# joeyee/Onet

Measured on AMD Instinct MI355X. Metric: training images/sec (twin 256x256 pass), higher is better.
Workload: dtype f32

## Files before the change

### onet_amd/csrc/conv_split.hip

```cpp
#include <algorithm>
#include <cstdlib>
#include "common.hpp"

using namespace onet;

typedef float f32x16 __attribute__((ext_vector_type(16)));
typedef __bf16 bf16x8 __attribute__((ext_vector_type(8)));
typedef __bf16 bf16x2 __attribute__((ext_vector_type(2)));
typedef unsigned int u32x4s __attribute__((ext_vector_type(4)));
typedef float f32x4s __attribute__((ext_vector_type(4)));

namespace {

constexpr unsigned OOB_S = 0x80000000u;

__device__ __forceinline__ __amdgpu_buffer_rsrc_t s_rsrc(const void* base, int64_t bytes) {
    const int n = bytes > 0x7fffffffll ? 0x7fffffff : (int)bytes;
    return __builtin_amdgcn_make_buffer_rsrc(const_cast<void*>(base), 0, n, 0x00020000);
}
__device__ __forceinline__ void split2(float a, float b, unsigned& hi, unsigned& mid) {
    const bf16x2 h = {(__bf16)a, (__bf16)b};
    const bf16x2 m = {(__bf16)(a - (float)h[0]), (__bf16)(b - (float)h[1])};
    hi = __builtin_bit_cast(unsigned, h);
    mid = __builtin_bit_cast(unsigned, m);
// ... 693 lines not shown
            }
#pragma unroll
            for (int idx = 0; idx < 9; ++idx) {
                const int kx = idx / 3, ky = idx % 3;
                if (idx < 8) {
                    const int nt = ((idx + 1) % 3) * 3 + (idx + 1) / 3;
#pragma unroll
                    for (int m = 0; m < 2; ++m) {
                        Aq[(idx + 1) & 1][m][0] = ab[nt * 2 * CO_T + m * 32];
                        Aq[(idx + 1) & 1][m][1] = ab[nt * 2 * CO_T + m * 32 + W_PART];
                    }
                }
                if (kx < 2) {
#pragma unroll
                    for (int j = 0; j < NB; ++j)
                        if (j % 3 == ky) {
                            Bq[(kx + 1) & 1][j][0] = bb[j * IN_COLS + kx + 1];
                            Bq[(kx + 1) & 1][j][1] = bb[j * IN_COLS + kx + 1 + IN_PART];
                        }
                }
                if (idx == 0) advance();
                {
                    constexpr int NPIECE = NII + NWI, PER = (NPIECE + C::LAST_TAP) / (C::LAST_TAP + 1);
#pragma unroll
                    for (int q = 0; q < PER; ++q) {
                        const int pc = idx * PER + q;
                        if (idx <= C::LAST_TAP && pc < NPIECE) {
                            if (pc & 1) { if (pc / 2 < NWI) dma_w(buf ^ 1, pc / 2); else dma_in(buf ^ 1, pc - NWI); }
                            else { if (pc / 2 < NII) dma_in(buf ^ 1, pc / 2); else dma_w(buf ^ 1, pc - NII); }
                        }
                    }
                }
                __builtin_amdgcn_sched_barrier(0);
#pragma unroll
                for (int m = 0; m < 2; ++m)
#pragma unroll
                    for (int n = 0; n < NT; ++n) {
                        if constexpr (PM == 2) {
                            const bf16x8 a0 = __builtin_bit_cast(bf16x8, Aq[idx & 1][m][0]), a1 = __builtin_bit_cast(bf16x8, Aq[idx & 1][m][1]);
                            const bf16x8 b0 = __builtin_bit_cast(bf16x8, Bq[kx & 1][n + ky][0]), b1 = __builtin_bit_cast(bf16x8, Bq[kx & 1][n + ky][1]);
                            acc[m][n] = __builtin_amdgcn_mfma_f32_32x32x16_bf16(a0, b0, acc[m][n], 0, 0, 0);
                            acc[m][n] = __builtin_amdgcn_mfma_f32_32x32x16_bf16(a1, b1, acc[m][n], 0, 0, 0);
                        } else if constexpr (F16) {
                            const f16x8 ah = __builtin_bit_cast(f16x8, Aq[idx & 1][m][0]), am = __builtin_bit_cast(f16x8, Aq[idx & 1][m][1]);
                            const f16x8 bh = __builtin_bit_cast(f16x8, Bq[kx & 1][n + ky][0]), bm = __builtin_bit_cast(f16x8, Bq[kx & 1][n + ky][1]);
                            acc[m][n] = __builtin_amdgcn_mfma_f32_32x32x16_f16(am, bh, acc[m][n], 0, 0, 0);
                            acc[m][n] = __builtin_amdgcn_mfma_f32_32x32x16_f16(ah, bm, acc[m][n], 0, 0, 0);
                            acc[m][n] = __builtin_amdgcn_mfma_f32_32x32x16_f16(ah, bh, acc[m][n], 0, 0, 0);
                        } else {
                            const bf16x8 ah = __builtin_bit_cast(bf16x8, Aq[idx & 1][m][0]), am = __builtin_bit_cast(bf16x8, Aq[idx & 1][m][1]);
                            const bf16x8 bh = __builtin_bit_cast(bf16x8, Bq[kx & 1][n + ky][0]), bm = __builtin_bit_cast(bf16x8, Bq[kx & 1][n + ky][1]);
                            acc[m][n] = __builtin_amdgcn_mfma_f32_32x32x16_bf16(am, bh, acc[m][n], 0, 0, 0);
                            acc[m][n] = __builtin_amdgcn_mfma_f32_32x32x16_bf16(ah, bm, acc[m][n], 0, 0, 0);
                            acc[m][n] = __builtin_amdgcn_mfma_f32_32x32x16_bf16(ah, bh, acc[m][n], 0, 0, 0);
                        }
                    }
                __builtin_amdgcn_sched_barrier(0);
            }
            asm volatile("s_waitcnt vmcnt(0)" ::: "memory");
            __syncthreads();
            buf ^= 1;
        }

#pragma unroll
        for (int m = 0; m < 2; ++m)
#pragma unroll
            for (int n = 0; n < NT; ++n)
#pragma unroll
                for (int r = 0; r < 16; ++r) acc[m][n][r] *= acc_scale;
        const auto [co0, tx, ty, b, y0, x0] = sp_tile(tile, a.coTiles, a.tilesX, a.tilesY);
        if constexpr (ST) {
            float* sc = reinterpret_cast<float*>(lds + 2 * BUF);
            constexpr float npw = (float)(NT * 32), inv_npw = 1.f / npw;
#pragma unroll
            for (int m = 0; m < 2; ++m)
#pragma unroll
                for (int r = 0; r < 16; ++r) {
                    const int piv = __builtin_bit_cast(int, acc[m][0][r]);
                    const float p0 = __builtin_bit_cast(float, __builtin_amdgcn_readlane(piv, 0));
                    const float p1 = __builtin_bit_cast(float, __builtin_amdgcn_readlane(piv, 32));
                    const float pv = kh ? p1 : p0;
                    float s1 = 0.f, s2 = 0.f;
#pragma unroll
                    for (int n = 0; n < NT; ++n) {
                        const float d = acc[m][n][r] - pv;
                        s1 += d;
                        s2 = fmaf(d, d, s2);
                    }
                    s1 = sp_half_sum(s1);
                    s2 = sp_half_sum(s2);
                    if (l31 == 31) {
                        const int cl = m * 32 + (r & 3) + 8 * (r >> 2) + 4 * kh;
                        sc[(wn * 64 + cl) * 2] = fmaf(s1, inv_npw, pv);
                        sc[(wn * 64 + cl) * 2 + 1] = fmaxf(fmaf(-s1 * inv_npw, s1, s2), 0.f);
                    }
                }
            __syncthreads();
            if (tid < 64 && co0 + tid < a.Cout) {
                float mw[8], qw[8];
#pragma unroll
                for (int w = 0; w < 8; ++w) {
                    mw[w] = sc[(w * 64 + tid) * 2];
                    qw[w] = sc[(w * 64 + tid) * 2 + 1];
                }
                const float mean = 0.125f * (((mw[0] + mw[1]) + (mw[2] + mw[3])) + ((mw[4] + mw[5]) + (mw[6] + mw[7])));
                float m2 = ((qw[0] + qw[1]) + (qw[2] + qw[3])) + ((qw[4] + qw[5]) + (qw[6] + qw[7]));
#pragma unroll
                for (int w = 0; w < 8; ++w) m2 = fmaf(npw * (mw[w] - mean), mw[w] - mean, m2);
                const int64_t nblk = (int64_t)a.B * a.tilesY * a.tilesX;
                const int64_t blk = ((int64_t)b * a.tilesY + ty) * a.tilesX + tx;
                float* sp = a.stats + ((int64_t)(co0 + tid) * nblk + blk) * 3;
                sp[0] = 8.f * npw;
                sp[1] = mean;
                sp[2] = m2;
            }
            __syncthreads();
        }
        float* zb = a.z + (int64_t)(W16 ? 2 * b + (l31 >> 4) : b) * a.z_bs;
        const int xo = W16 ? (l31 & 15) : x0 + l31;
        if constexpr (ACT) {
            const float* cf = act_cf + cf_par * 192;
            float vmax = 0.f;
#pragma unroll
            for (int m = 0; m < 2; ++m)
#pragma unroll
                for (int g = 0; g < 4; ++g) {
                    const int cl = m * 32 + 8 * g + 4 * kh;
                    const f32x4s mean = *reinterpret_cast<const f32x4s*>(cf + cl);
                    const f32x4s sc = *reinterpret_cast<const f32x4s*>(cf + 64 + cl);
                    const f32x4s sh = *reinterpret_cast<const f32x4s*>(cf + 128 + cl);
#pragma unroll
                    for (int n = 0; n < NT; ++n)
#pragma unroll
                        for (int j = 0; j < 4; ++j) {
                            const float v = fmaxf(fmaf(acc[m][n][4 * g + j] - mean[j], sc[j], sh[j]), 0.f);
                            acc[m][n][4 * g + j] = v;
                            vmax = fmaxf(vmax, v);
                        }
                }
            if (a.act_amax) {
#pragma unroll
                for (int o = 32; o > 0; o >>= 1) vmax = fmaxf(vmax, __shfl_xor(vmax, o, 64));
                if (lane == 0 && vmax == vmax)
                    atomicMax(a.act_amax + ((tile * NWV + wn) & (AMAX_SLOTS - 1)) * AMAX_STRIDE, __builtin_bit_cast(unsigned, vmax));
            }
            if (a.act_a) {
                float* ab = a.act_a + (int64_t)b * a.act_a_bs;
#pragma unroll
                for (int m = 0; m < 2; ++m)
#pragma unroll
                    for (int n = 0; n < NT; ++n) {
                        const int yo = y0 + wn * NT + n;
                        if (yo < a.H && xo < a.W) {
#pragma unroll
                            for (int r = 0; r < 16; ++r) {
                                const int co = co0 + m * 32 + (r & 3) + 8 * (r >> 2) + 4 * kh;
                                if (co < a.Cout) ab[(int64_t)co * HW + (int64_t)yo * a.W + xo] = acc[m][n][r];
                            }
                        }
                    }
            }
        }
        if constexpr (PM == 1 && !ST && !W16) {
            if (ACT || (a.zP && co0 >= a.zP_ch0)) {
                const float zs = zP_scale;
                u32x4s* zp = reinterpret_cast<u32x4s*>(reinterpret_cast<unsigned*>(a.zP) + (int64_t)b * a.zP_bs);
#pragma unroll
                for (int m = 0; m < 2; ++m)
#pragma unroll
                    for (int n = 0; n < NT; ++n) {
                        const int yo = y0 + wn * NT + n;
#pragma unroll
                        for (int e = 0; e < 2; ++e) {
                            float v[8];
#pragma unroll
                            for (int j = 0; j < 4; ++j) {
                                const float f0 = acc[m][n][8 * e + j], f1 = acc[m][n][8 * e + 4 + j];
                                const unsigned d0 = __builtin_bit_cast(unsigned, f0);
                                const unsigned d1 = __builtin_bit_cast(unsigned, f1);
                                const auto sw = __builtin_amdgcn_permlane32_swap(d0, d1, false, false);
                                const unsigned lo = sw[0], hi4 = sw[1];
                                v[j] = __builtin_bit_cast(float, lo);
                                v[4 + j] = __builtin_bit_cast(float, hi4);
                            }
                            u32x4s hi, mid;
#pragma unroll
                            for (int k = 0; k < 4; ++k) {
                                unsigned hh, mm;
                                split2h_s(v[2 * k], v[2 * k + 1], zs, hh, mm);
                                hi[k] = hh;
                                mid[k] = mm;
                            }
                            if (yo < a.H && xo < a.W) {
                                const int c8 = ((co0 - a.zP_ch0 + m * 32) >> 3) + 2 * e + kh;
                                u32x4s* d = zp + ((int64_t)(c8 * a.H + yo) * 2) * a.W + xo;
                                d[0] = hi;
                                d[a.W] = mid;
                            }
                        }
                    }
                continue;
            }
        }
#pragma unroll
        for (int m = 0; m < 2; ++m)
#pragma unroll
            for (int n = 0; n < NT; ++n) {
                const int yo = y0 + wn * NT + n;
                if (yo < a.H && xo < a.W) {
#pragma unroll
                    for (int r = 0; r < 16; ++r) {
                        const int co = co0 + m * 32 + (r & 3) + 8 * (r >> 2) + 4 * kh;
                        if (co < a.Cout) zb[(int64_t)co * HW + (int64_t)yo * a.W + xo] = acc[m][n][r];
                    }
                }
            }
    }
}


template <bool ST, int PM, bool W16, bool RD = false>
__global__ __launch_bounds__(512, 2) void conv3x3_pre16_kernel(SpPreArgs a) {
    constexpr bool F16 = PM == 1;
    using C = SpPreCfg<W16>;
    static_assert(C::NW == 8 && C::NT == 2, "conv3x3_pre16_kernel: 8 waves of 2 rows");
    constexpr int NT = 2, IN_COLS = C::IN_COLS, NWI = C::NWI, CO_T = C::CO_T, NPIXP = C::NPIXP;
    constexpr int BUF = C::BUF_SLOTS, IN_PART = C::IN_PART;
    constexpr int NII = (2 * IN_PART + 511) / 512;
    constexpr int CH_OFF = W16 ? 18 : 16;
    constexpr int NSTEP = PM == 2 ? 9 : 14;
    extern __shared__ __attribute__((aligned(16))) unsigned char smem_s[];
    u32x4s* lds = reinterpret_cast<u32x4s*>(smem_s);

    int t_first, t_end, t_stride;
    sp_tile_range(a.tilesX * a.tilesY * a.B * a.coTiles, t_first, t_end, t_stride);
    if (t_first >= t_end) return;

    const int tid = threadIdx.x, lane = tid & 63, wn = __builtin_amdgcn_readfirstlane(tid >> 6);
    const int r16 = lane & 15, lq = lane >> 4, hq = lq & 1, gq = lq >> 1;
    const int HW = a.H * a.W;
    const int nchunks = PM == 2 ? a.Cin >> 5 : a.Cin >> 4;

    const i32x4s wr = sp_rsrc4(a.wq, (int64_t)a.Cin * (PM == 2 ? 1 : 2) * 9 * a.Cout * 2);
    float xs_inv = 1.f, xs_inv2 = 1.f;
    (void)amax_scale(amax_read(a.x_slots), a.x_always != 0, xs_inv);
    (void)amax_scale(amax_read(a.x_slots2), a.x_always != 0, xs_inv2);
    const int split_chunk = a.split_ch ? (PM == 2 ? a.split_ch >> 5 : a.split_ch >> 4) : 0;
    const float grp_ratio = split_chunk ? xs_inv / xs_inv2 : 1.f;
    const float acc_scale = (split_chunk ? xs_inv2 : xs_inv) * (F16 ? reinterpret_cast<const float*>(a.wq + (int64_t)a.Cin * 2 * 9 * a.Cout)[1] : 1.f);
    const unsigned in_step = (unsigned)(16 * HW * 4), w_step = (unsigned)(2 * 9 * 2 * a.Cout * 16);
    const unsigned lds0 = (unsigned)(uintptr_t)(__attribute__((address_space(3))) unsigned char*)smem_s;

    unsigned in_off[NII], w_off[NWI];
    i32x4s xr;
    int st_tile = t_first, st_chunk = 0;
    unsigned cin_bytes = 0, cw_bytes = 0;
    auto setup_stage = [&]() __attribute__((always_inline)) {
        const bool live = st_tile < t_end;
        const auto [co0, tx, ty, b, y0, x0] = sp_tile(live ? st_tile : t_first, a.coTiles, a.tilesX, a.tilesY);
        xr = sp_rsrc4(reinterpret_cast<const unsigned*>(a.xs) + (int64_t)(W16 ? 2 * b : b) * a.xs_bs,
                      (W16 ? a.xs_bs * 4 : 0) + (int64_t)a.Cin * HW * (PM == 2 ? 2 : 4));
#pragma unroll
        for (int k = 0; k < NII; ++k) {
            const int i = (wn + 8 * k) * 64 + lane;
            const int ph = i / NPIXP, pix = i % NPIXP;
            const int r = pix / IN_COLS, c = pix % IN_COLS;
            const int img = W16 ? c / 18 : 0;
            const int yy = y0 - 1 + r, xx = W16 ? c % 18 - 1 : x0 - 1 + c;
            const bool ok = live && i < 2 * IN_PART && pix < C::NPIX && yy >= 0 && yy < a.H && xx >= 0 && xx < a.W;
            const unsigned io = W16 ? (unsigned)(img * a.xs_bs * 4) : 0u;
            in_off[k] = !ok ? OOB_S : PM == 2 ? io + (unsigned)(((ph * a.H + yy) * a.W + xx) * 16)
                                              : io + (unsigned)(((((ph & 1) * a.H + yy) * 2 + (ph >> 1)) * a.W + xx) * 16);
        }
#pragma unroll
        for (int k = 0; k < NWI; ++k) {
            const int i = tid + 512 * k;
            const int co = i & (CO_T - 1), pth = i >> 6;
            const bool ok = live && (i < C::W_SLOTS) && (co0 + co < a.Cout);
            w_off[k] = ok ? (unsigned)((pth * a.Cout + co0 + co) * 16) : OOB_S;
        }
    };
    auto advance = [&]() __attribute__((always_inline)) {
        ++st_chunk;
        cin_bytes += in_step;
        cw_bytes += w_step;
        if (st_chunk == nchunks) {
            st_chunk = 0;
            cin_bytes = cw_bytes = 0;
            st_tile += t_stride;
            setup_stage();
        }
    };
    auto dma_in = [&](int buf, int k) __attribute__((always_inline)) {
        if ((wn + 8 * k) * 64 < 2 * IN_PART)
            sp_dma16(xr, lds0 + (unsigned)((buf * BUF + C::W_SLOTS + (wn + 8 * k) * 64) * 16), in_off[k], cin_bytes);
    };
    auto dma_w = [&](int buf, int k) __attribute__((always_inline)) {
        if (k < NWI - 1 || wn < (C::W_SLOTS - 512 * (NWI - 1)) / 64)
            sp_dma16(wr, lds0 + (unsigned)((buf * BUF + (wn + 8 * k) * 64) * 16), w_off[k], cw_bytes);
    };

    const int xrow0 = (wn * NT) * IN_COLS + r16;
    const u32x4s* const xa_p = lds + C::W_SLOTS + (PM == 2 ? lq : hq) * NPIXP + xrow0;
    const u32x4s* const xh_p = lds + C::W_SLOTS + (2 + hq) * NPIXP + xrow0 + gq;
    const u32x4s* const xv_p = lds + C::W_SLOTS + (2 + hq) * NPIXP + xrow0 + gq * IN_COLS + 2;
    const u32x4s* const xs_p = lds + C::W_SLOTS + (2 + hq) * NPIXP + xrow0 + 2;
    const u32x4s* const wa_p = lds + (gq * 9 * 2 + hq) * CO_T + r16;
    const u32x4s* const wh_p = lds + (gq * 2 + hq) * CO_T + r16;
    const u32x4s* const wv_p = lds + ((3 * gq + 2) * 2 + hq) * CO_T + r16;
    const u32x4s* const ws_p = gq == 0 ? lds + (8 * 2 + hq) * CO_T + r16 : lds + C::W_SLOTS + C::NPIX;
    const int ws_ct = gq == 0 ? 16 : 0;

    setup_stage();
#pragma unroll
    for (int k = 0; k < NII; ++k) dma_in(0, k);
#pragma unroll
    for (int k = 0; k < NWI; ++k) dma_w(0, k);
    asm volatile("s_waitcnt vmcnt(0)" ::: "memory");
    __syncthreads();
    int buf = 0;
    for (int tile = t_first; tile < t_end; tile += t_stride) {
        f32x4s acc[4][NT][2];
#pragma unroll
        for (int ct = 0; ct < 4; ++ct)
#pragma unroll
            for (int n = 0; n < NT; ++n)
#pragma unroll
                for (int ch = 0; ch < 2; ++ch) acc[ct][n][ch] = f32x4s{0.f, 0.f, 0.f, 0.f};

        for (int c = 0; c < nchunks; ++c) {
            if (split_chunk && c == split_chunk && grp_ratio != 1.f) {
#pragma unroll
                for (int ct = 0; ct < 4; ++ct)
#pragma unroll
                    for (int n = 0; n < NT; ++n)
#pragma unroll
                        for (int ch = 0; ch < 2; ++ch) acc[ct][n][ch] *= grp_ratio;
            }
            const int bo = buf * BUF;
            u32x4s Xp[2][NT + 2][2], Wf[2][4];
            auto load_x = [&](int ph, int f) __attribute__((always_inline)) {
                const int j = f >> 1, ch = f & 1, p = ph & 1;
                if (ph < 3) Xp[p][j][ch] = xa_p[bo + j * IN_COLS + ch * CH_OFF + ph];
                else if (ph == 3) Xp[p][j][ch] = xh_p[bo + j * IN_COLS + ch * CH_OFF];
                else if (j < NT) Xp[p][j][ch] = xv_p[bo + j * IN_COLS + ch * CH_OFF];
                else Xp[p][j][ch] = xs_p[bo + j * IN_COLS + ch * CH_OFF];
            };
            auto load_w = [&](int s) __attribute__((always_inline)) {
#pragma unroll
                for (int ct = 0; ct < 4; ++ct) {
                    if (s < 9) Wf[s & 1][ct] = wa_p[bo + ((s % 3) * 3 + s / 3) * 2 * CO_T + ct * 16];
                    else if (s < 12) Wf[s & 1][ct] = wh_p[bo + (s - 9) * 6 * CO_T + ct * 16];
                    else if (s == 12) Wf[s & 1][ct] = wv_p[bo + ct * 16];
                    else Wf[s & 1][ct] = ws_p[bo + ct * ws_ct];
                }
            };
#pragma unroll
            for (int f = 0; f < 2 * (NT + 2); ++f) load_x(0, f);
            load_w(0);
#pragma unroll
            for (int s = 0; s < NSTEP; ++s) {
                const int ph = s < 9 ? s / 3 : (s < 12 ? 3 : 4);
                const int ro = s < 9 ? s % 3 : (s < 12 ? s - 9 : (s == 12 ? 0 : NT));
                if (s + 1 < NSTEP) load_w(s + 1);
                if (s < 12 && ph + 1 < (PM == 2 ? 3 : 5)) {
#pragma unroll
                    for (int f = 0; f < 2 * (NT + 2); ++f)
                        if (f % 3 == s % 3) load_x(ph + 1, f);
                }
                if (s == 0) advance();
                {
                    constexpr int NPIECE = NII + NWI, PER = (NPIECE + C::LAST_TAP) / (C::LAST_TAP + 1);
#pragma unroll
                    for (int q = 0; q < PER; ++q) {
                        const int pc = s * PER + q;
                        if (s <= C::LAST_TAP && pc < NPIECE) {
                            if (pc & 1) { if (pc / 2 < NWI) dma_w(buf ^ 1, pc / 2); else dma_in(buf ^ 1, pc - NWI); }
                            else { if (pc / 2 < NII) dma_in(buf ^ 1, pc / 2); else dma_w(buf ^ 1, pc - NII); }
                        }
                    }
                }
                __builtin_amdgcn_sched_barrier(0);
#pragma unroll
                for (int ct = 0; ct < 4; ++ct)
#pragma unroll
                    for (int n = 0; n < NT; ++n)
#pragma unroll
                        for (int ch = 0; ch < 2; ++ch) {
                            if constexpr (F16)
                                acc[ct][n][ch] = __builtin_amdgcn_mfma_f32_16x16x32_f16(__builtin_bit_cast(f16x8, Xp[ph & 1][ro + n][ch]),
                                                                                        __builtin_bit_cast(f16x8, Wf[s & 1][ct]), acc[ct][n][ch], 0, 0, 0);
                            else
                                acc[ct][n][ch] = __builtin_amdgcn_mfma_f32_16x16x32_bf16(__builtin_bit_cast(bf16x8, Xp[ph & 1][ro + n][ch]),
                                                                                         __builtin_bit_cast(bf16x8, Wf[s & 1][ct]), acc[ct][n][ch], 0, 0, 0);
                        }
                __builtin_amdgcn_sched_barrier(0);
            }
            asm volatile("s_waitcnt vmcnt(0)" ::: "memory");
            __syncthreads();
            buf ^= 1;
        }

#pragma unroll
        for (int ct = 0; ct < 4; ++ct)
#pragma unroll
            for (int n = 0; n < NT; ++n)
#pragma unroll
                for (int ch = 0; ch < 2; ++ch) acc[ct][n][ch] *= acc_scale;
        const auto [co0, tx, ty, b, y0, x0] = sp_tile(tile, a.coTiles, a.tilesX, a.tilesY);
        if constexpr (ST) {
            float* sc = reinterpret_cast<float*>(lds + (buf ^ 1) * BUF);
            constexpr float npw = (float)(NT * 32);
#pragma unroll
            for (int ct = 0; ct < 4; ++ct) {
                const float pv = acc[ct][0][0][0];
                float s1 = 0.f, s2 = 0.f;
#pragma unroll
                for (int n = 0; n < NT; ++n)
#pragma unroll
                    for (int ch = 0; ch < 2; ++ch)
#pragma unroll
                        for (int r = 0; r < 4; ++r) {
                            const float d = acc[ct][n][ch][r] - pv;
                            s1 += d;
                            s2 = fmaf(d, d, s2);
                        }
                float mean = fmaf(s1, 1.f / 16.f, pv), m2 = fmaxf(fmaf(-s1 * (1.f / 16.f), s1, s2), 0.f), cnt = 16.f;
#pragma unroll
                for (int o = 16; o <= 32; o <<= 1) {
                    const float mo = __shfl_xor(mean, o, 64), qo = __shfl_xor(m2, o, 64);
                    const float dlt = mo - mean;
                    m2 = (m2 + qo) + (0.5f * cnt) * dlt * dlt;
                    mean = 0.5f * (mean + mo);
                    cnt *= 2.f;
                }
                if (lq == 0) {
                    sc[(wn * 64 + ct * 16 + r16) * 2] = mean;
                    sc[(wn * 64 + ct * 16 + r16) * 2 + 1] = m2;
                }
            }
            __syncthreads();
            if (tid < 64 && co0 + tid < a.Cout) {
                float mw[8], qw[8];
#pragma unroll
                for (int w = 0; w < 8; ++w) {
                    mw[w] = sc[(w * 64 + tid) * 2];
                    qw[w] = sc[(w * 64 + tid) * 2 + 1];
                }
                const float mean = 0.125f * (((mw[0] + mw[1]) + (mw[2] + mw[3])) + ((mw[4] + mw[5]) + (mw[6] + mw[7])));
                float m2 = ((qw[0] + qw[1]) + (qw[2] + qw[3])) + ((qw[4] + qw[5]) + (qw[6] + qw[7]));
#pragma unroll
                for (int w = 0; w < 8; ++w) m2 = fmaf(npw * (mw[w] - mean), mw[w] - mean, m2);
                const int64_t nblk = (int64_t)a.B * a.tilesY * a.tilesX;
                const int64_t blk = ((int64_t)b * a.tilesY + ty) * a.tilesX + tx;
                float* sp = a.stats + ((int64_t)(co0 + tid) * nblk + blk) * 3;
                sp[0] = 8.f * npw;
                sp[1] = mean;
                sp[2] = m2;
            }
            __syncthreads();
        }
        f32x4s zr[4][NT][2];
        const float* rd_sv = nullptr;
        if constexpr (RD) {
            const int img0 = W16 ? 2 * b : b;
            rd_sv = a.rd_save + (int64_t)(a.rd_gimg ? img0 / a.rd_gimg : 0) * 4 * a.Cout;
#pragma unroll
            for (int ct = 0; ct < 4; ++ct)
#pragma unroll
                for (int n = 0; n < NT; ++n)
#pragma unroll
                    for (int ch = 0; ch < 2; ++ch) {
                        const int co = co0 + ct * 16 + r16, yo = y0 + wn * NT + n, xo = (W16 ? 0 : x0 + 16 * ch) + 4 * lq;
                        f32x4s zz = {0.f, 0.f, 0.f, 0.f};
                        if (co < a.Cout && yo < a.H && xo < a.W) {
                            const int64_t zo = (int64_t)(W16 ? img0 + ch : img0) * a.rd_z_bs + (int64_t)co * HW + (int64_t)yo * a.W + xo;
                            if (a.rd_z16) {
                                const uint2 u = *reinterpret_cast<const uint2*>(reinterpret_cast<const __bf16*>(a.rd_z) + zo);
                                zz = f32x4s{__builtin_bit_cast(float, u.x << 16), __builtin_bit_cast(float, u.x & 0xffff0000u),
                                            __builtin_bit_cast(float, u.y << 16), __builtin_bit_cast(float, u.y & 0xffff0000u)};
                            } else {
                                zz = *reinterpret_cast<const f32x4s*>(a.rd_z + zo);
                            }
                        }
                        zr[ct][n][ch] = zz;
                    }
            __builtin_amdgcn_sched_barrier(0);
        }
        {
            const int half = r16 >> 3, c8 = r16 & 7;
            float* zb = a.z + (int64_t)(W16 ? 2 * b + half : b) * a.z_bs;
            const int xo = (W16 ? 0 : x0 + 16 * half) + 4 * lq;
#pragma unroll
            for (int n = 0; n < NT; ++n) {
                const int yo = y0 + wn * NT + n;
#pragma unroll
                for (int ct = 0; ct < 4; ++ct) {
                    const i32x4s va = __builtin_bit_cast(i32x4s, acc[ct][n][0]), vb = __builtin_bit_cast(i32x4s, acc[ct][n][1]);
                    const i32x4s e1 = {__builtin_amdgcn_update_dpp(va.x, vb.x, 0x128, 0xf, 0xc, false), __builtin_amdgcn_update_dpp(va.y, vb.y, 0x128, 0xf, 0xc, false),
                                       __builtin_amdgcn_update_dpp(va.z, vb.z, 0x128, 0xf, 0xc, false), __builtin_amdgcn_update_dpp(va.w, vb.w, 0x128, 0xf, 0xc, false)};
                    const i32x4s e2 = {__builtin_amdgcn_update_dpp(vb.x, va.x, 0x128, 0xf, 0x3, false), __builtin_amdgcn_update_dpp(vb.y, va.y, 0x128, 0xf, 0x3, false),
                                       __builtin_amdgcn_update_dpp(vb.z, va.z, 0x128, 0xf, 0x3, false), __builtin_amdgcn_update_dpp(vb.w, va.w, 0x128, 0xf, 0x3, false)};
                    const f32x4s d1 = __builtin_bit_cast(f32x4s, e1), d2 = __builtin_bit_cast(f32x4s, e2);
                    if constexpr (PM == 2 && !ST && !W16 && !RD) {
                        if (a.zP && co0 >= a.zP_ch0) {
                            const unsigned a0 = pack2bf(d1[0], d1[1]), a1 = pack2bf(d1[2], d1[3]);
                            const unsigned b0 = pack2bf(d2[0], d2[1]), b1 = pack2bf(d2[2], d2[3]);
                            const bool o1 = (c8 & 1) != 0, o2 = (c8 & 2) != 0, o4 = (c8 & 4) != 0;
                            auto st1 = [&](unsigned x) {
                                const unsigned y = (unsigned)__shfl_xor((int)x, 1, 64);
                                return o1 ? ((y >> 16) | (x & 0xffff0000u)) : ((x & 0xffffu) | (y << 16));
                            };
                            const unsigned A0 = st1(a0), A1 = st1(a1), B0 = st1(b0), B1 = st1(b1);
                            const unsigned ra = (unsigned)__shfl_xor((int)(o2 ? A0 : A1), 2, 64), rb = (unsigned)__shfl_xor((int)(o2 ? B0 : B1), 2, 64);
                            const unsigned ka = o2 ? A1 : A0, kb = o2 ? B1 : B0;
                            const unsigned Alo = o2 ? ra : ka, Ahi = o2 ? ka : ra, Blo = o2 ? rb : kb, Bhi = o2 ? kb : rb;
                            const unsigned r0 = (unsigned)__shfl_xor((int)(o4 ? Alo : Blo), 4, 64), r1 = (unsigned)__shfl_xor((int)(o4 ? Ahi : Bhi), 4, 64);
                            const u32x4s slot = o4 ? u32x4s{r0, r1, Blo, Bhi} : u32x4s{Alo, Ahi, r0, r1};
                            const int xs = x0 + 16 * half + 4 * lq + (c8 & 3);
                            if (yo < a.H && xs < a.W) {
                                const int g8 = ((co0 - a.zP_ch0) >> 3) + 2 * ct + (o4 ? 1 : 0);
                                u32x4s* zp = reinterpret_cast<u32x4s*>(reinterpret_cast<unsigned*>(a.zP) + (int64_t)b * a.zP_bs);
                                zp[((int64_t)g8 * a.H + yo) * a.W + xs] = slot;
                            }
                            continue;
                        }
                    }
                    if (yo < a.H && xo < a.W) {
                        const int co = co0 + ct * 16 + c8;
                        const int64_t off = (int64_t)co * HW + (int64_t)yo * a.W + xo;
                        if (a.z16) {
                            __bf16* o = reinterpret_cast<__bf16*>(a.z) + (int64_t)(W16 ? 2 * b + half : b) * a.z_bs + off;
                            const bf16x2 p0 = {(__bf16)d1[0], (__bf16)d1[1]}, p1 = {(__bf16)d1[2], (__bf16)d1[3]};
                            const bf16x2 q0 = {(__bf16)d2[0], (__bf16)d2[1]}, q1 = {(__bf16)d2[2], (__bf16)d2[3]};
                            if (co < a.Cout) *reinterpret_cast<uint2*>(o) = uint2{__builtin_bit_cast(unsigned, p0), __builtin_bit_cast(unsigned, p1)};
                            if (co + 8 < a.Cout) *reinterpret_cast<uint2*>(o + (int64_t)8 * HW) = uint2{__builtin_bit_cast(unsigned, q0), __builtin_bit_cast(unsigned, q1)};
                        } else {
                            float* o = zb + off;
                            if (co < a.Cout) *reinterpret_cast<f32x4s*>(o) = d1;
                            if (co + 8 < a.Cout) *reinterpret_cast<f32x4s*>(o + (int64_t)8 * HW) = d2;
                        }
                    }
                }
            }
        }
        if constexpr (RD) {
            __builtin_amdgcn_sched_barrier(0);
            float* sc = reinterpret_cast<float*>(lds + (buf ^ 1) * BUF);
            float vmax = 0.f;
#pragma unroll
            for (int ct = 0; ct < 4; ++ct) {
                const int co = co0 + ct * 16 + r16, cc = min(co, a.Cout - 1);
                const float mean = rd_sv[cc], invstd = rd_sv[a.Cout + cc], scl = rd_sv[2 * a.Cout + cc], sh = rd_sv[3 * a.Cout + cc];
                float s1 = 0.f, s2 = 0.f;
#pragma unroll
                for (int n = 0; n < NT; ++n)
#pragma unroll
                    for (int ch = 0; ch < 2; ++ch) {
                        const int yo = y0 + wn * NT + n, xo = (W16 ? 0 : x0 + 16 * ch) + 4 * lq;
                        if (co < a.Cout && yo < a.H && xo < a.W) {
#pragma unroll
                            for (int r = 0; r < 4; ++r) {
                                const float da = acc[ct][n][ch][r], d = zr[ct][n][ch][r] - mean;
                                const float dy = fmaf(d, scl, sh) > 0.f ? da : 0.f;
                                s1 += dy;
                                s2 = fmaf(dy, d * invstd, s2);
                                vmax = fmaxf(vmax, fabsf(da));
                            }
                        }
                    }
                s1 += __shfl_xor(s1, 16, 64);
                s2 += __shfl_xor(s2, 16, 64);
                s1 += __shfl_xor(s1, 32, 64);
                s2 += __shfl_xor(s2, 32, 64);
                if (lq == 0) {
                    sc[(wn * 64 + ct * 16 + r16) * 2] = s1;
                    sc[(wn * 64 + ct * 16 + r16) * 2 + 1] = s2;
                }
            }
            if (a.rd_amax) {
#pragma unroll
                for (int o = 32; o > 0; o >>= 1) vmax = fmaxf(vmax, __shfl_xor(vmax, o, 64));
                if (lane == 0 && vmax == vmax) atomicMax(a.rd_amax + ((blockIdx.x * 8 + wn) & (AMAX_SLOTS - 1)) * AMAX_STRIDE, __builtin_bit_cast(unsigned, vmax));
            }
            __syncthreads();
            if (tid < 64 && co0 + tid < a.Cout) {
                double t1 = 0.0, t2 = 0.0;
#pragma unroll
                for (int w = 0; w < 8; ++w) {
                    t1 += (double)sc[(w * 64 + tid) * 2];
                    t2 += (double)sc[(w * 64 + tid) * 2 + 1];
                }
                const int64_t blk = ((int64_t)b * a.tilesY + ty) * a.tilesX + tx;
                float* o = a.rd_rec + (blk * a.Cout + co0 + tid) * 4;
                o[0] = (float)t1;
                o[1] = (float)(t1 - (double)o[0]);
                o[2] = (float)t2;
                o[3] = (float)(t2 - (double)o[2]);
            }
            __syncthreads();
        }
    }
}

template <class Args>
int sp_launch_persistent(void (*kern)(Args), PerDeviceOnce& once, int lds_bytes, int64_t tiles, int block, const char* name, const Args& a, hipStream_t st) {
    if (once.first()) {
        (void)hipFuncSetAttribute(reinterpret_cast<const void*>(kern), hipFuncAttributeMaxDynamicSharedMemorySize, lds_bytes);
    }
    const int64_t resident = (int64_t)device_cu_count();
    const int64_t blocks = std::min<int64_t>((tiles + 7) / 8 * 8, std::max<int64_t>(8, resident / 8 * 8));
    hipLaunchKernelGGL(kern, dim3((unsigned)blocks), dim3(block), lds_bytes, st, a);
    return check_launch(name);
}

template <bool ST, int PM, bool W16, bool RD = false, bool ACT = false>
int launch_split_pre(SpPreArgs a, hipStream_t st) {
    using C = SpPreCfg<W16>;
    const int LDS_BYTES = C::LDS_BYTES + (ST ? C::NW * 64 * 2 * 4 : 0) + (ACT ? 2 * 3 * 64 * 4 : 0);
    a.tilesX = W16 ? 1 : cdiv(a.W, C::TW);
    a.tilesY = cdiv(a.H, C::ROWS);
    a.coTiles = cdiv(a.Cout, C::CO_T);
    if (W16) a.B /= 2;
    const int64_t tiles = (int64_t)a.B * a.tilesX * a.tilesY * a.coTiles;
    ONET_REQUIRE(tiles > 0 && tiles < (1ll << 31), "conv3x3_split_pre: tile count %lld out of range", (long long)tiles);
    constexpr bool P16 = RD || PM == 2 || (ST && !W16);
    void (*kern)(SpPreArgs);
    if constexpr (P16) kern = conv3x3_pre16_kernel<ST, PM, W16, RD>;
    else kern = conv3x3_split_pre_kernel<ST, PM, W16, ACT>;
    static PerDeviceOnce attr_once;
    return sp_launch_persistent(kern, attr_once, LDS_BYTES, tiles, C::NW * 64, ACT ? "conv3x3_split_pre_act_kernel" : "conv3x3_split_pre_kernel", a, st);
}

int split_nparts(int B, int H, int W) {
    if (B <= 0 || W < 32 || (W % SpCfg::TW) || (H % SpCfg::ROWS)) return 0;
    const int64_t n = (int64_t)B * (H / SpCfg::ROWS) * (W / SpCfg::TW);
    return n < (1 << 30) ? (int)n : 0;
}

template <bool ST, bool NORM, bool F16>
int launch_split(SpArgs a, hipStream_t st) {
    using C = SpCfg;
    const int LDS_BYTES = C::LDS_BYTES + (ST ? C::NW * 64 * 2 * 4 : 0) + (NORM ? 2 * 2 * 8 * 4 * 4 : 0);
    a.tilesX = cdiv(a.W, C::TW);
    a.tilesY = cdiv(a.H, C::ROWS);
    a.coTiles = cdiv(a.Cout, C::CO_T);
    const int64_t tiles = (int64_t)a.B * a.tilesX * a.tilesY * a.coTiles;
    ONET_REQUIRE(tiles > 0 && tiles < (1ll << 31), "conv3x3_split: tile count %lld out of range", (long long)tiles);
    static PerDeviceOnce attr_once;
    return sp_launch_persistent(conv3x3_split_kernel<ST, NORM, F16>, attr_once, LDS_BYTES, tiles, 512, "conv3x3_split_kernel", a, st);
}

int split_fwd(const float* x, int64_t x_bs, const void* wq, float* z, int64_t z_bs, int B, int Cin, int Cout, int H, int W,
              void* stream, float* stats, int wq_f16, const float* nsave = nullptr, int n_groups = 0, const unsigned* x_amax = nullptr,
              int x_always = 0) {
    ONET_REQUIRE(x && wq && z, "conv3x3_split_fwd: null pointer");
    ONET_REQUIRE(B > 0 && Cin > 0 && Cout > 0 && H > 0 && W > 16, "conv3x3_split_fwd: bad shape (maps wider than 16 pixels)");
    ONET_REQUIRE((Cin % 16) == 0, "conv3x3_split_fwd: Cin must be a multiple of 16 (use onet_conv_fwd)");
    ONET_REQUIRE((W & 3) == 0 && (x_bs & 3) == 0 && (reinterpret_cast<uintptr_t>(x) & 15) == 0,
                 "conv3x3_split_fwd: W %% 4 == 0 and 16-byte aligned image rows required (use onet_conv3x3_winograd4_fwd)");
    ONET_REQUIRE(x_bs >= (int64_t)Cin * H * W && z_bs >= (int64_t)Cout * H * W, "conv3x3_split_fwd: batch stride too small");
    ONET_REQUIRE((int64_t)(Cin + 32) * H * W * 4 < (1ll << 31) && (int64_t)(Cin + 32) * 2 * 9 * Cout * 2 < (1ll << 31),
                 "conv3x3_split_fwd: operand exceeds the 2 GiB buffer-resource range");
    SpArgs a{x, x_bs, (const __bf16*)wq, z, z_bs, B, Cin, Cout, H, W, 0, 0, 0, stats, nsave, 1, x_amax, x_always};
    ONET_REQUIRE(!x_amax || wq_f16, "conv3x3_split: magnitude slots go with the fp16 pack");
    if (stats) ONET_REQUIRE(split_nparts(B, H, W) > 0, "conv3x3_split_fwd_stats: the map must be made of full 16 x 32 tiles");
    if (nsave) {
        ONET_REQUIRE(n_groups > 0 && B % n_groups == 0, "conv3x3_split_fwd_norm: the batch must hold n_groups equal statistics groups");
        a.nimg = B / n_groups;
        if (wq_f16) return stats ? launch_split<true, true, true>(a, as_stream(stream)) : launch_split<false, true, true>(a, as_stream(stream));
        return stats ? launch_split<true, true, false>(a, as_stream(stream)) : launch_split<false, true, false>(a, as_stream(stream));
    }
    if (wq_f16) return stats ? launch_split<true, false, true>(a, as_stream(stream)) : launch_split<false, false, true>(a, as_stream(stream));
    return stats ? launch_split<true, false, false>(a, as_stream(stream)) : launch_split<false, false, false>(a, as_stream(stream));
}


struct SwArgs {
    const float* x;
    int64_t x_bs;
    const float* dz;
    int64_t dz_bs;
    float* slab;
    int B, Cin, Cout, H, W, ciTiles, coTiles, splitK, tilesX;
    const float* nsave;
    int nimg;
    const unsigned* x_amax;
    const unsigned* dz_amax;
};

constexpr int SR_SDZ = 36;
template <int G> struct SwCfg {
    static constexpr int SPG = 8 / G;
    static constexpr int P = G == 1 ? 36 : (G == 2 ? 20 : 12);
    static constexpr int SLOT = G * P;
    static constexpr int SX = 4 * SLOT + 4;
    static constexpr int X_PART = 64 * SX;
// ... 858 lines not shown
```

Baseline: 592.4.

## Reorder split-precision conv MFMA steps to reuse hi/mid input fragments across taps

For the non-PM==2 path, the MFMA step schedule is reordered so that the hi and mid input fragments for a row offset stay in registers and are reused across paired weight sets. Input loads for the vertical and skip terms are scattered at fixed steps, and the LDS pointer bases move to index the partition by an explicit IN_PART/W_PART offset. The aim is fewer LDS reads of input fragments per chunk and better overlap of loads with MFMAs. The cost is a more intricate hand-written schedule, a risk of higher register pressure, and an implicit dependence on the LDS layout of the partitions.

```diff
diff --git a/onet_amd/csrc/conv_split.hip b/onet_amd/csrc/conv_split.hip
--- a/onet_amd/csrc/conv_split.hip
+++ b/onet_amd/csrc/conv_split.hip
@@ -1019,9 +1019,9 @@
 
     const int xrow0 = (wn * NT) * IN_COLS + r16;
     const u32x4s* const xa_p = lds + C::W_SLOTS + (PM == 2 ? lq : hq) * NPIXP + xrow0;
-    const u32x4s* const xh_p = lds + C::W_SLOTS + (2 + hq) * NPIXP + xrow0 + gq;
-    const u32x4s* const xv_p = lds + C::W_SLOTS + (2 + hq) * NPIXP + xrow0 + gq * IN_COLS + 2;
-    const u32x4s* const xs_p = lds + C::W_SLOTS + (2 + hq) * NPIXP + xrow0 + 2;
+    const u32x4s* const xh_p = lds + C::W_SLOTS + hq * NPIXP + xrow0 + gq;
+    const u32x4s* const xv_p = lds + C::W_SLOTS + hq * NPIXP + xrow0 + gq * IN_COLS + 2;
+    const u32x4s* const xs_p = lds + C::W_SLOTS + hq * NPIXP + xrow0 + 2;
     const u32x4s* const wa_p = lds + (gq * 9 * 2 + hq) * CO_T + r16;
     const u32x4s* const wh_p = lds + (gq * 2 + hq) * CO_T + r16;
     const u32x4s* const wv_p = lds + ((3 * gq + 2) * 2 + hq) * CO_T + r16;
@@ -1057,33 +1057,68 @@
             const int bo = buf * BUF;
             u32x4s Xp[2][NT + 2][2], Wf[2][4];
             auto load_x = [&](int ph, int f) __attribute__((always_inline)) {
-                const int j = f >> 1, ch = f & 1, p = ph & 1;
-                if (ph < 3) Xp[p][j][ch] = xa_p[bo + j * IN_COLS + ch * CH_OFF + ph];
-                else if (ph == 3) Xp[p][j][ch] = xh_p[bo + j * IN_COLS + ch * CH_OFF];
-                else if (j < NT) Xp[p][j][ch] = xv_p[bo + j * IN_COLS + ch * CH_OFF];
-                else Xp[p][j][ch] = xs_p[bo + j * IN_COLS + ch * CH_OFF];
+                const int j = f >> 1, ch = f & 1;
+                Xp[ph & 1][j][ch] = xa_p[bo + j * IN_COLS + ch * CH_OFF + ph];
             };
             auto load_w = [&](int s) __attribute__((always_inline)) {
 #pragma unroll
+                for (int ct = 0; ct < 4; ++ct) Wf[s & 1][ct] = wa_p[bo + ((s % 3) * 3 + s / 3) * 2 * CO_T + ct * 16];
+            };
+            auto load_xh = [&](int p, int f) __attribute__((always_inline)) {
+                const int j = f >> 1, ch = f & 1;
+                Xp[p][j][ch] = xh_p[bo + p * IN_PART + j * IN_COLS + ch * CH_OFF];
+            };
+            auto load_xvs = [&](int p, int j) __attribute__((always_inline)) {
+#pragma unroll
+                for (int ch = 0; ch < 2; ++ch) {
+                    if (j < NT) Xp[p][j][ch] = xv_p[bo + p * IN_PART + j * IN_COLS + ch * CH_OFF];
+                    else Xp[p][j][ch] = xs_p[bo + p * IN_PART + j * IN_COLS + ch * CH_OFF];
+                }
+            };
+            auto load_wset = [&](int k) __attribute__((always_inline)) {
+#pragma unroll
                 for (int ct = 0; ct < 4; ++ct) {
-                    if (s < 9) Wf[s & 1][ct] = wa_p[bo + ((s % 3) * 3 + s / 3) * 2 * CO_T + ct * 16];
-                    else if (s < 12) Wf[s & 1][ct] = wh_p[bo + (s - 9) * 6 * CO_T + ct * 16];
-                    else if (s == 12) Wf[s & 1][ct] = wv_p[bo + ct * 16];
-                    else Wf[s & 1][ct] = ws_p[bo + ct * ws_ct];
+                    if (k < 6) Wf[k & 1][ct] = wh_p[bo + (k & 1) * C::W_PART + (k >> 1) * 6 * CO_T + ct * 16];
+                    else if (k < 8) Wf[k & 1][ct] = wv_p[bo + (k & 1) * C::W_PART + ct * 16];
+                    else if (k == 8) Wf[k & 1][ct] = wa_p[bo + 8 * 2 * CO_T + ct * 16];
+                    else Wf[k & 1][ct] = ws_p[bo + ct * ws_ct];
                 }
             };
-#pragma unroll
-            for (int f = 0; f < 2 * (NT + 2); ++f) load_x(0, f);
-            load_w(0);
+            if constexpr (PM == 2) {
+#pragma unroll
+                for (int f = 0; f < 2 * (NT + 2); ++f) load_x(0, f);
+                load_w(0);
+            } else {
+#pragma unroll
+                for (int f = 0; f < 2 * (NT + 2); ++f) load_xh(0, f);
+                load_wset(0);
+            }
 #pragma unroll
             for (int s = 0; s < NSTEP; ++s) {
-                const int ph = s < 9 ? s / 3 : (s < 12 ? 3 : 4);
-                const int ro = s < 9 ? s % 3 : (s < 12 ? s - 9 : (s == 12 ? 0 : NT));
-                if (s + 1 < NSTEP) load_w(s + 1);
-                if (s < 12 && ph + 1 < (PM == 2 ? 3 : 5)) {
-#pragma unroll
-                    for (int f = 0; f < 2 * (NT + 2); ++f)
-                        if (f % 3 == s % 3) load_x(ph + 1, f);
+                const int g3 = s / 3, t3 = s % 3;
+                const int wk = s < 12 ? 2 * g3 + (t3 == 2) : s - 4;
+                const int pool = PM == 2 ? g3 & 1 : (s < 12 ? t3 == 1 : s - 12);
+                const int ro = PM == 2 ? t3 : (s < 9 ? g3 : (s < 12 ? 0 : NT));
+                const int wb = PM == 2 ? s & 1 : wk & 1;
+                if constexpr (PM == 2) {
+                    if (s + 1 < NSTEP) load_w(s + 1);
+                    if (g3 + 1 < 3) {
+#pragma unroll
+                        for (int f = 0; f < 2 * (NT + 2); ++f)
+                            if (f % 3 == t3) load_x(g3 + 1, f);
+                    }
+                } else {
+                    if (s == 0) {
+#pragma unroll
+                        for (int f = 0; f < 2 * (NT + 2); ++f) load_xh(1, f);
+                    }
+                    if ((s >= 12 || t3 != 1) && wk + 1 < 10) load_wset(wk + 1);
+                    if (s == 4) load_xvs(0, 0);
+                    if (s == 5) load_xvs(1, 0);
+                    if (s == 7) { load_xvs(0, 1); load_xvs(1, 1); }
+                    if (s == 9) load_xvs(0, 2);
+                    if (s == 10) { load_xvs(0, 3); load_xvs(1, 2); }
+                    if (s == 11) load_xvs(1, 3);
                 }
                 if (s == 0) advance();
                 {
@@ -1105,11 +1140,11 @@
 #pragma unroll
                         for (int ch = 0; ch < 2; ++ch) {
                             if constexpr (F16)
-                                acc[ct][n][ch] = __builtin_amdgcn_mfma_f32_16x16x32_f16(__builtin_bit_cast(f16x8, Xp[ph & 1][ro + n][ch]),
-                                                                                        __builtin_bit_cast(f16x8, Wf[s & 1][ct]), acc[ct][n][ch], 0, 0, 0);
+                                acc[ct][n][ch] = __builtin_amdgcn_mfma_f32_16x16x32_f16(__builtin_bit_cast(f16x8, Xp[pool][ro + n][ch]),
+                                                                                        __builtin_bit_cast(f16x8, Wf[wb][ct]), acc[ct][n][ch], 0, 0, 0);
                             else
-                                acc[ct][n][ch] = __builtin_amdgcn_mfma_f32_16x16x32_bf16(__builtin_bit_cast(bf16x8, Xp[ph & 1][ro + n][ch]),
-                                                                                         __builtin_bit_cast(bf16x8, Wf[s & 1][ct]), acc[ct][n][ch], 0, 0, 0);
+                                acc[ct][n][ch] = __builtin_amdgcn_mfma_f32_16x16x32_bf16(__builtin_bit_cast(bf16x8, Xp[pool][ro + n][ch]),
+                                                                                         __builtin_bit_cast(bf16x8, Wf[wb][ct]), acc[ct][n][ch], 0, 0, 0);
                         }
                 __builtin_amdgcn_sched_barrier(0);
             }
```

Measured after the change: 594.7 (median of 6 runs). About the same (+0.4%).
